# happyxtt/CNNs_SLFP_quantization

Measured on AMD Instinct MI355X. Metric: images/sec at batch 256, MobileNetV1 SLFP<3,4> ImageNet-224; % HBM roofline, higher is better.
Workload: dtype f32 (1x1 contraction: fp16 MFMA operands, f32 accumulate); 1 GPU; mobilenetv1_imagenet224: all 27 Conv2d_Q layers, SLFP<3,4> Qbits=8, NHWC, batch 256 per GPU as 2 concurrent image groups of 128 on 2 HIP streams, inputs resident in HBM; batch_per_gpu=256, global_batch=256, parallelism=batch-sharded x1, one-time RCCL broadcast of the u8 weight codes, pointwise_mfma=pw_mfma_f16x1

## Files before the change

cnns_slfp_quantization_amd/_lib.py:

```python
import ctypes
import os

_HERE = os.path.dirname(os.path.abspath(__file__))
LIB_PATH = os.path.join(_HERE, "libslfp_hip.so")

OK, ERR_BAD_ARG, ERR_SHAPE, ERR_UNSUPPORTED, ERR_ALIGNMENT, ERR_HIP = 0, -1, -2, -3, -4, -5
FMT_ACT8, FMT_W8, FMT_SFP7, FMT_EXT = 0, 1, 2, 4
LAYOUT_NCHW, LAYOUT_NHWC = 0, 1
BWD_DENSE = 1
MFMA_DEFAULT, MFMA_F16X1, MFMA_F16X3 = 0, 1, 3
OPT_SGD, OPT_DSGD, OPT_SSGD = 0, 1, 2

SYMBOLS = (
    "slfp_version", "slfp_last_error", "slfp_device_count",
    "slfp_encode_f32", "slfp_decode_f32", "slfp_quantize_f32", "slfp_quantize_layerout_f32", "slfp_absmax_f32",
    "slfp_conv2d_out_shape", "slfp_conv2d_kernel_name", "slfp_conv2d_wprep_bytes",
    "slfp_conv2d_prepare_weights", "slfp_conv2d_prepare_weights_codes", "slfp_conv2d_workspace_bytes", "slfp_conv2d_fwd", "slfp_conv2d_fwd_post",
    "slfp_linear_workspace_bytes", "slfp_linear_fwd", "slfp_linear_prepare_weights", "slfp_linear_fwd_prepared",
    "slfp_nchw_to_nhwc_f32", "slfp_nhwc_to_nchw_f32", "slfp_debug_div_mismatches",
    "slfp_debug_enc_mismatches", "slfp_enc_table_ok", "slfp_dwpw_supported", "slfp_dwpw_fwd",
    "slfp_conv2d_codes_supported", "slfp_conv2d_fwd_codes", "slfp_conv2d_fwd_codes_ws", "slfp_maxpool2d_codes", "slfp_debug_code_mismatches", "slfp_debug_reload_switches",
    "slfp_debug_enc_hl_mismatches", "slfp_sgd_step_f32", "slfp_debug_dw3x3_variant",
    "slfp_conv2d_bwd_supported", "slfp_conv2d_bwd_kernel_name", "slfp_conv2d_bwd_workspace_bytes", "slfp_conv2d_bwd",
    "slfp_conv2d_bwd_supported_ex", "slfp_conv2d_bwd_kernel_name_ex", "slfp_conv2d_bwd_workspace_bytes_ex", "slfp_conv2d_bwd_ex",
    "slfp_conv2d_res_supported", "slfp_conv2d_fwd_res",
    "slfp_conv2d_codes_slice_supported", "slfp_conv2d_fwd_codes_slice", "slfp_maxpool2d_codes_ex", "slfp_maxpool2d_out_shape",
    "slfp_conv2d_entry_supported", "slfp_conv2d_fwd_entry",
)


class ConvDesc(ctypes.Structure):
    _fields_ = [
        ("n", ctypes.c_int64), ("c_in", ctypes.c_int64), ("h", ctypes.c_int64), ("w", ctypes.c_int64),
        ("c_out", ctypes.c_int64), ("kh", ctypes.c_int64), ("kw", ctypes.c_int64),
        ("stride_h", ctypes.c_int32), ("stride_w", ctypes.c_int32), ("pad_h", ctypes.c_int32),
        ("pad_w", ctypes.c_int32), ("dil_h", ctypes.c_int32), ("dil_w", ctypes.c_int32),
        ("groups", ctypes.c_int32), ("x_layout", ctypes.c_int32), ("y_layout", ctypes.c_int32),
# ... 33 lines not shown
    L = ctypes.CDLL(LIB_PATH)
    vp, sz, ci, cf, i64 = ctypes.c_void_p, ctypes.c_size_t, ctypes.c_int, ctypes.c_float, ctypes.c_int64
    dp = ctypes.POINTER(ConvDesc)
    sigs = {
        "slfp_version": (ci, []),
        "slfp_last_error": (ctypes.c_char_p, []),
        "slfp_device_count": (ci, []),
        "slfp_encode_f32": (ci, [vp, vp, sz, cf, ci, vp]),
        "slfp_decode_f32": (ci, [vp, vp, sz, ci, vp]),
        "slfp_quantize_f32": (ci, [vp, vp, sz, cf, ci, vp]),
        "slfp_quantize_layerout_f32": (ci, [vp, vp, sz, vp]),
        "slfp_absmax_f32": (ci, [vp, sz, vp, vp]),
        "slfp_conv2d_out_shape": (ci, [dp, ctypes.POINTER(i64), ctypes.POINTER(i64)]),
        "slfp_conv2d_kernel_name": (ctypes.c_char_p, [dp]),
        "slfp_debug_dw3x3_variant": (ctypes.c_char_p, [dp, ci]),
        "slfp_conv2d_wprep_bytes": (sz, [dp]),
        "slfp_conv2d_prepare_weights": (ci, [dp, vp, vp, vp, vp]),
        "slfp_conv2d_prepare_weights_codes": (ci, [dp, vp, vp, vp, vp]),
        "slfp_conv2d_workspace_bytes": (sz, [dp]),
        "slfp_conv2d_fwd": (ci, [dp, vp, vp, vp, vp, vp, vp, vp]),
        "slfp_conv2d_fwd_post": (ci, [dp, vp, vp, vp, vp, vp, ci, vp, vp, vp, vp]),
        "slfp_linear_workspace_bytes": (sz, [i64, i64, i64]),
        "slfp_linear_fwd": (ci, [vp, vp, vp, vp, i64, i64, i64, cf, cf, ci, ci, vp, vp]),
        "slfp_linear_prepare_weights": (ci, [vp, vp, i64, i64, cf, ci, ci, vp]),
        "slfp_linear_fwd_prepared": (ci, [vp, vp, vp, vp, i64, i64, i64, cf, cf, ci, ci, vp]),
        "slfp_nchw_to_nhwc_f32": (ci, [vp, vp, i64, i64, i64, i64, vp]),
        "slfp_nhwc_to_nchw_f32": (ci, [vp, vp, i64, i64, i64, i64, vp]),
        "slfp_debug_div_mismatches": (ci, [cf, vp, vp]),
        "slfp_debug_enc_mismatches": (ci, [cf, ci, vp, vp]),
        "slfp_enc_table_ok": (ci, [cf, ci]),
# ... 48 lines not shown
```

cnns_slfp_quantization_amd/csrc/codec.hip:

```cpp
#include <cstdarg>
#include <mutex>
#include <map>
#include <set>
#include <utility>
#include <cstdio>
#include "slfp_device.hpp"
#include "slfp_enc.hpp"
#include "slfp_host.hpp"

namespace slfp {

static thread_local char g_err[512] = "";

void set_error(const char* fmt, ...) {
    va_list ap;
    va_start(ap, fmt);
    vsnprintf(g_err, sizeof(g_err), fmt, ap);
    va_end(ap);
}

int fail(int code, const char* fmt, ...) {
    va_list ap;
    va_start(ap, fmt);
    vsnprintf(g_err, sizeof(g_err), fmt, ap);
// ... 36 lines not shown
    e = std::getenv("SLFP_PW_NT_MIN_MB");
    w.pw_nt_min_mb = e ? atoll(e) : 0;
    e = std::getenv("SLFP_DW_NT_MIN_MB");
    w.dw_nt_min_mb = e ? atoll(e) : 30;
    w.stem_old = std::getenv("SLFP_STEM_OLD") != nullptr;
    w.pwc_slice = std::getenv("SLFP_PWC_NOSLICE") == nullptr;
    w.dense_generic = std::getenv("SLFP_DENSE_GENERIC") != nullptr;
    e = std::getenv("SLFP_DENSE_CFG");
    w.dense_cfg = e ? atoi(e) : 0;
    e = std::getenv("SLFP_DENSE_NWB");
    w.dense_nwb = e ? atoi(e) : 0;
    w.dense_res = std::getenv("SLFP_DENSE_NORES") == nullptr;
    w.dense_encx = std::getenv("SLFP_DENSE_NOENCX") == nullptr;
    w.stem_im2row = std::getenv("SLFP_STEM_IM2ROW") != nullptr;
    w.dw_rows = parse_dw_rows(std::getenv("SLFP_DW_ROWS"));
    e = std::getenv("SLFP_PW_STREAM_MAX_KB");
    w.pw_stream_max_kb = e ? atoi(e) : 30;
    return w;
}
static Switches g_switches = read_switches();
const Switches& switches() { return g_switches; }
void reload_switches() { g_switches = read_switches(); }

int device_cu_count() {
    static std::mutex mu;
    static std::map<int, int> cus;
    int dev = 0;
    if (hipGetDevice(&dev) != hipSuccess) { (void)hipGetLastError(); return 256; }
    std::lock_guard<std::mutex> lock(mu);
    const auto it = cus.find(dev);
// ... 305 lines not shown
```

cnns_slfp_quantization_amd/csrc/conv_abi.hip:

```cpp
#include <cstring>
#include "slfp_device.hpp"
#include "slfp_codes.hpp"
#include "slfp_host.hpp"

namespace slfp {

static size_t round256(size_t b) { return (b + 255) & ~(size_t)255; }

static int make_plan_core(const slfp_conv2d_desc* d, ConvPlan* plan) {
    if (!d || !plan) return fail(SLFP_ERR_BAD_ARG, "conv2d: null descriptor");
    if (d->n <= 0 || d->c_in <= 0 || d->h <= 0 || d->w <= 0 || d->c_out <= 0 || d->kh <= 0 || d->kw <= 0)
        return fail(SLFP_ERR_SHAPE, "conv2d: non-positive size");
    if (d->stride_h <= 0 || d->stride_w <= 0 || d->dil_h <= 0 || d->dil_w <= 0 || d->pad_h < 0 || d->pad_w < 0)
        return fail(SLFP_ERR_SHAPE, "conv2d: bad stride/dilation/padding");
    if (d->groups <= 0 || d->c_in % d->groups || d->c_out % d->groups)
        return fail(SLFP_ERR_SHAPE, "conv2d: groups=%d does not divide C_in=%lld / C_out=%lld", d->groups,
                    (long long)d->c_in, (long long)d->c_out);
    if (d->qbits != 8 && d->qbits != 7)
        return fail(SLFP_ERR_BAD_ARG, "conv2d: qbits must be 8 (SLFP<3,4>) or 7 (SFP<3,3>), got %d", d->qbits);
    if ((d->x_layout != SLFP_LAYOUT_NCHW && d->x_layout != SLFP_LAYOUT_NHWC) ||
        (d->y_layout != SLFP_LAYOUT_NCHW && d->y_layout != SLFP_LAYOUT_NHWC))
        return fail(SLFP_ERR_BAD_ARG, "conv2d: unknown layout");
    if (!(d->ka > 0.f) || !(d->kw_scale > 0.f)) return fail(SLFP_ERR_BAD_ARG, "conv2d: Ka and Kw must be > 0");
    if (!scale_div_ok(d->ka) || !scale_div_ok(d->kw_scale))
// ... 219 lines not shown
const char* slfp_conv2d_kernel_name(const slfp_conv2d_desc* d) {
    ConvPlan p;
    if (make_plan(d, &p) != SLFP_OK) return "invalid";
    return family_name(p, *d);
}

const char* slfp_debug_dw3x3_variant(const slfp_conv2d_desc* d, int has_post) {
    ConvPlan p;
    if (make_plan(d, &p) != SLFP_OK || p.family != kDw3x3) return "none";
    static const float one = 1.f;
    const PostOp post = {has_post ? &one : nullptr, has_post ? &one : nullptr, 0, 0};
    if (dw3x3_rows_applicable(*d, p, nullptr, post)) return "rows";
    return dw3x3_tile_applicable(*d, p, nullptr, post) ? "tile" : "general";
}

size_t slfp_conv2d_wprep_bytes(const slfp_conv2d_desc* d) {
    ConvPlan p;
    if (make_plan(d, &p) != SLFP_OK) return 0;
    return p.wprep_bytes;
}

int slfp_conv2d_prepare_weights(const slfp_conv2d_desc* d, const float* w_oihw, void* wprep, float* weight_q_oihw,
                                void* stream) {
    ConvPlan p;
    const int rc = make_plan(d, &p);
    if (rc != SLFP_OK) return rc;
    if (!w_oihw || !wprep) return fail(SLFP_ERR_BAD_ARG, "slfp_conv2d_prepare_weights: null pointer");
    if (!aligned16(wprep)) return fail(SLFP_ERR_ALIGNMENT, "slfp_conv2d_prepare_weights: wprep must be 16-byte aligned");
    return launch_prepare_weights(*d, p, w_oihw, wprep, weight_q_oihw, as_stream(stream));
}
// ... 394 lines not shown
```

cnns_slfp_quantization_amd/csrc/conv_pw.hip:

```cpp
#include <cstdlib>
#include "slfp_device.hpp"
#include "slfp_enc.hpp"
#include "slfp_codes.hpp"
#include "slfp_host.hpp"
#include "conv_pw_params.hpp"

namespace slfp {

__device__ __forceinline__ half8 enc_frag(const float4 a, const float4 b, const EncArgs& e, const unsigned char* tb) {
    const uint2 pa = enc4_f16_raw(a, e.r1, e.lo, e.hi, tb), pb = enc4_f16_raw(b, e.r1, e.lo, e.hi, tb);
    typedef uint32_t u32x4 __attribute__((ext_vector_type(4)));
    return __builtin_bit_cast(half8, u32x4{pa.x, pa.y, pb.x, pb.y});
}
__device__ __forceinline__ half8 enc_frag_nan(const float4 a, const float4 b, const EncArgs& e, const unsigned char* tb) {
    const uint2 pa = enc4_f16(a, e.r1, e.lo, e.hi, tb), pb = enc4_f16(b, e.r1, e.lo, e.hi, tb);
    typedef uint32_t u32x4 __attribute__((ext_vector_type(4)));
    return __builtin_bit_cast(half8, u32x4{pa.x, pa.y, pb.x, pb.y});
}

__device__ __forceinline__ void enc_frag_hl(const float4 a, const float4 b, const EncArgs& e, const unsigned char* tb,
                                            const unsigned char* tl, half8& h, half8& l) {
    typedef uint32_t u32x4 __attribute__((ext_vector_type(4)));
    uint32_t h0, h1, h2, h3, l0, l1, l2, l3;
    enc2_f16_hl(a.x, a.y, e.r1, e.lo, e.hi, tb, tl, h0, l0);
// ... 247 lines not shown
                float4 r = tile_out(j);
                if constexpr (RES) r = res_add(r, rc, p.post.relu);
                const int n = j * 16 + kq * 4;
                if constexpr (A8) {
                    if (live && n < p.N) *reinterpret_cast<float2*>(yr + j * 16) = make_float2(r.x, r.y);
                    if (live && n + 2 < p.N) *reinterpret_cast<float2*>(yr + j * 16 + 2) = make_float2(r.z, r.w);
                } else {
                    if (live && n < p.N) st_stream4<SLFP_NT_PW>(yr + j * 16, r);
                }
            }
        }
    }
}


template <int FMT, int PASSES, int WM, int WN, int MT, int NT, bool KFULL, bool TAB = false, bool STG = false, bool RES = false, bool YC = false>
__global__ __launch_bounds__(64 * WM * WN, (WM * WN) <= 4 ? 2 : 4) void k_pw_tiled(const PwParams p) {
    static_assert(!STG || NT == 4, "the staged epilogue stores a wave's 64 channels per row");
    static_assert(!RES || STG, "residual operand: staged epilogue only");
    static_assert(!YC || (TAB && !STG && !RES && PASSES == 1 && NT == 4), "code output: single-pass table kernels, four channel tiles per wave");
    constexpr int TABB = TAB ? kPwTab : 64;
    constexpr int TABL = (TAB && (PASSES == 3 || YC)) ? kPwTab : 16;
    constexpr int T = 64 * WM * WN;
    constexpr int BM = WM * MT * 16;
    constexpr int BN = WN * NT * 16;
    constexpr int NLD = BM * 16 / T;
    static_assert(BM * 16 % T == 0, "staging must divide evenly");
    constexpr int XBYTES = BM * 128;

    __shared__ __attribute__((aligned(16))) unsigned char stab[TABB];
    __shared__ __attribute__((aligned(16))) unsigned char stab_lo[TABL];
    extern __shared__ __attribute__((aligned(16))) unsigned char smem[];
    uint32_t* sT = reinterpret_cast<uint32_t*>(stab);
    unsigned char* xs = smem;
    if constexpr (TAB) enc_fill<T>(reinterpret_cast<uint2*>(stab), p.enc);
    else lut_fill<FMT>(sT);
    if constexpr (TAB && (PASSES == 3 || YC)) enc_fill_compact<T>(reinterpret_cast<uint2*>(stab_lo), p.enc_lo);

    const uint32_t b = xcd_remap(blockIdx.x, p.nblocks);
    const uint32_t nb = b % p.n_blocks, mb = b / p.n_blocks;
    const int64_t m0 = (int64_t)mb * p.rb;
    const int lane = threadIdx.x & 63, wave = threadIdx.x >> 6;
    const int wm = wave / WN, wn = wave % WN;
    const int col = lane & 15, kq = lane >> 4;

    const int kc = threadIdx.x & 15;
    const int st_chunk = (kc >> 3) * 4 + (kc & 3);
    const uint32_t st_sub = (uint32_t)((kc & 7) >> 2) * 8u;
    const float* src[NLD];
#pragma unroll
    for (int i = 0; i < NLD; ++i) {
        const int row = (threadIdx.x >> 4) + i * (T / 16);
        int64_t m = m0 + (row < p.rb ? row : p.rb - 1);
        m = m < p.M ? m : p.M - 1;
        src[i] = p.x + x_row_offset(p, m) + kc * 4;
    }

    float4 st[NLD];
    auto load_stage = [&](int t) {
#ifdef SLFP_ABL_NOX
        if (t >= 2) {
#pragma unroll
            for (int i = 0; i < NLD; ++i) asm volatile("" : "+v"(st[i].x), "+v"(st[i].y), "+v"(st[i].z), "+v"(st[i].w));
            return;
        }
#endif
#pragma unroll
        for (int i = 0; i < NLD; ++i) {
            if constexpr (KFULL) {
                st[i] = ld_stream4<SLFP_NT_PWT>(src[i] + t * 64);
            } else {
                const int k = t * 64 + kc * 4;
                const int kk = k < p.K ? t * 64 : p.K - 4 - kc * 4;
                st[i] = *reinterpret_cast<const float4*>(src[i] + kk);
                if (k >= p.K) st[i] = make_float4(0.f, 0.f, 0.f, 0.f);
            }
        }
    };
    auto encode_store = [&](int buf) {
        unsigned char* hi = xs + (size_t)buf * (PASSES == 3 ? 2 : 1) * XBYTES;
        unsigned char* lo = hi + XBYTES;
#pragma unroll
        for (int i = 0; i < NLD; ++i) {
            const int row = (threadIdx.x >> 4) + i * (T / 16);
            const uint32_t off = lds_x_off(row, st_chunk) + st_sub;
            if constexpr (TAB && PASSES == 3) {
                uint2 ph, pl;
                enc2_f16_hl(st[i].x, st[i].y, p.enc.r1, p.enc.lo, p.enc.hi, stab, stab_lo, ph.x, pl.x);
                enc2_f16_hl(st[i].z, st[i].w, p.enc.r1, p.enc.lo, p.enc.hi, stab, stab_lo, ph.y, pl.y);
                if (__builtin_expect(enc_has_nan4(st[i]), 0)) enc_patch_nan4_f16(st[i], ph);
                *reinterpret_cast<uint2*>(hi + off) = ph;
                *reinterpret_cast<uint2*>(lo + off) = pl;
            } else if constexpr (TAB) {
#ifdef SLFP_ABL_NOENC
// ... 23 lines not shown
    const int ntile0 = (int)nb * (BN / 16) + wn * NT;
    const size_t wplane = (size_t)(p.wlo - p.whi);
    const int wn_u = __builtin_amdgcn_readfirstlane(wn);
    const int ntile0u = (int)nb * (BN / 16) + wn_u * NT;
    const uint64_t wbytes = (uint64_t)p.n_tiles * p.KS * 1024;
    const uint32_t wrecs = (uint32_t)(wbytes > 0xFFFFFFFFull ? 0xFFFFFFFFull : wbytes);
    const __amdgpu_buffer_rsrc_t rwh = __builtin_amdgcn_make_buffer_rsrc(const_cast<_Float16*>(p.whi), 0, wrecs, 0x00020000);
    const __amdgpu_buffer_rsrc_t rwl = __builtin_amdgcn_make_buffer_rsrc(const_cast<_Float16*>(PASSES == 3 ? p.wlo : p.whi), 0, wrecs, 0x00020000);
    uint32_t wsoff[NT];
#pragma unroll
    for (int j = 0; j < NT; ++j) {
        const int nt = ntile0u + j < p.n_tiles ? ntile0u + j : p.n_tiles - 1;
        wsoff[j] = (uint32_t)nt * (uint32_t)p.KS * 1024u;
    }
    const uint32_t wvoff = (uint32_t)lane * 16u;
    half8 wh[NT], wl[NT];
    auto load_w = [&](int kstep) {
#ifdef SLFP_ABL_NOW
        if (kstep >= 1) {
#pragma unroll
            for (int j = 0; j < NT; ++j) asm volatile("" : "+v"(wh[j]));
            return;
        }
#endif
#pragma unroll
        for (int j = 0; j < NT; ++j) {
            typedef uint32_t u32x4w __attribute__((ext_vector_type(4)));
            const uint32_t so = wsoff[j] + (uint32_t)kstep * 1024u;
            wh[j] = __builtin_bit_cast(half8, __builtin_amdgcn_raw_buffer_load_b128(rwh, wvoff, so, 0));
            if constexpr (PASSES == 3) wl[j] = __builtin_bit_cast(half8, __builtin_amdgcn_raw_buffer_load_b128(rwl, wvoff, so, 0));
        }
    };
    auto mfma_step = [&](int buf, int ks) {
        const unsigned char* hi = xs + (size_t)buf * (PASSES == 3 ? 2 : 1) * XBYTES;
        const unsigned char* lo = hi + XBYTES;
#pragma unroll
        for (int i = 0; i < MT; ++i) {
            const int row = (wm * MT + i) * 16 + col;
            const uint32_t off = lds_x_off(row, ks * 4 + kq);
            const half8 xh = *reinterpret_cast<const half8*>(hi + off);
            half8 xl;
            if constexpr (PASSES == 3) xl = *reinterpret_cast<const half8*>(lo + off);
#pragma unroll
            for (int j = 0; j < NT; ++j) {
                if constexpr (PASSES == 3) {
                    acc[i][j] = __builtin_amdgcn_mfma_f32_16x16x32_f16(wl[j], xh, acc[i][j], 0, 0, 0);
                    acc[i][j] = __builtin_amdgcn_mfma_f32_16x16x32_f16(wh[j], xl, acc[i][j], 0, 0, 0);
                }
#ifdef SLFP_ABL_NOMFMA
                asm volatile("" :: "v"(wh[j]), "v"(xh));
#else
                acc[i][j] = __builtin_amdgcn_mfma_f32_16x16x32_f16(wh[j], xh, acc[i][j], 0, 0, 0);
#endif
            }
        }
    };

    SLFP_STAMP(0);
    __syncthreads();
    SLFP_STAMP(1);
    load_stage(0);
    encode_store(0);
    load_stage(KT > 1 ? 1 : 0);
    __syncthreads();
    SLFP_STAMP(2);

    for (int t = 0; t + 1 < KT; ++t) {
        const int buf = t & 1;
#ifdef SLFP_PW_STAMPS2
        if (t == 3) SLFP_STAMP(3);
#endif
        load_w(t * 2);
        encode_store(buf ^ 1);
        load_stage(t + 2 < KT ? t + 2 : KT - 1);
#ifdef SLFP_PW_STAMPS2
        if (t == 3) { asm volatile("s_waitcnt lgkmcnt(0)" ::: "memory"); SLFP_STAMP(4); }
#endif
        mfma_step(buf, 0);
#ifdef SLFP_PW_STAMPS2
        if (t == 3) { asm volatile("s_nop 0" : "+v"(acc[0][0]), "+v"(acc[3][3])); SLFP_STAMP(5); }
#endif
        load_w(t * 2 + 1);
        mfma_step(buf, 1);
#ifdef SLFP_PW_STAMPS2
        if (t == 3) { asm volatile("s_nop 0" : "+v"(acc[0][0]), "+v"(acc[3][3])); SLFP_STAMP(6); }
#endif
        __syncthreads();
#ifdef SLFP_PW_STAMPS2
        if (t == 3) SLFP_STAMP(7);
#else
        SLFP_STAMP(3 + (t < 8 ? t : 8));
#endif
    }
    SLFP_STAMP(12);
    const int srow = lane >> 4, sch = lane & 15;
    const int n_st = ntile0 * 16 + sch * 4;
    const uint64_t yleft = (uint64_t)(p.M - m0) * p.N * 4;
    const uint32_t ybytes = (uint32_t)(yleft > 0xFFFFFFFFull ? 0xFFFFFFFFull : yleft);
    auto piece = [&](int i, int h) {
        const int row = (wm * MT + i) * 16 + h * 4 + srow;
        const bool ok = row < p.rb && m0 + row < p.M && n_st < p.N;
        return ok ? (uint32_t)(row * p.N + n_st) * 4u : 0xFFFFFFF0u;
    };
    const __amdgpu_buffer_rsrc_t rr = __builtin_amdgcn_make_buffer_rsrc(const_cast<float*>(RES ? p.res : p.y) + (size_t)m0 * p.N, 0, ybytes, 0x00020000);
    u32x4r rq[4];
    {
        const int t = KT - 1, buf = t & 1;
        load_w(t * 2);
        mfma_step(buf, 0);
        load_w(t * 2 + 1);
        if constexpr (RES) {
#pragma unroll
            for (int h = 0; h < 4; ++h) rq[h] = res_load_stg(rr, piece(0, h));
        }
        mfma_step(buf, 1);
    }

    const int n_lo = (int)nb * BN;
    float* lsc = reinterpret_cast<float*>(xs);
    float* lsh = lsc + BN;
    if (p.post.scale) {
        __syncthreads();
        for (int i = threadIdx.x; i < BN; i += T) {
            const bool in = n_lo + i < p.N;
            lsc[i] = in ? p.post.scale[n_lo + i] : 1.f;
            lsh[i] = in ? p.post.shift[n_lo + i] : 0.f;
        }
        __syncthreads();
    }
    SLFP_STAMP(13);
    if constexpr (YC) {
        const float r1 = p.enc_lo.r1, lo = p.enc_lo.lo, hi = p.enc_lo.hi;
#pragma unroll
        for (int i = 0; i < MT; ++i) {
            uint32_t c[NT];
#pragma unroll
            for (int j = 0; j < NT; ++j) {
// ... 7 lines not shown
                    r.z = __builtin_fmaf(r.z, sc.z, sh.z); r.w = __builtin_fmaf(r.w, sc.w, sh.w);
                }
                if (p.sgn) c[j] = code_sign4(enc4_code<false>(r, r1, lo, hi, stab_lo), r, p.fmt_out);
                else c[j] = enc4_code_relu(relu_of_nan4(r), r1, lo, hi, stab_lo);
            }
            rows_transpose4(c[0], c[1], c[2], c[3]);
            const int row = (wm * MT + i) * 16 + col;
            const int n = (ntile0 + kq) * 16;
            typedef uint32_t u32x4 __attribute__((ext_vector_type(4)));
            if (row < p.rb && m0 + row < p.M && n < p.N)
                *reinterpret_cast<u32x4*>(p.yc + (size_t)(m0 + row) * p.N + n) = u32x4{c[0], c[1], c[2], c[3]};
        }
        return;
    }
    if constexpr (STG) {
        unsigned char* stg = xs + 2 * (PASSES == 3 ? 2 : 1) * XBYTES + wave * (16 * kStgRow);
        const __amdgpu_buffer_rsrc_t ry = __builtin_amdgcn_make_buffer_rsrc(p.y + (size_t)m0 * p.N, 0, ybytes, 0x00020000);
#pragma unroll
        for (int i = 0; i < MT; ++i) {
#pragma unroll
            for (int j = 0; j < NT; ++j) {
                const int n = (ntile0 + j) * 16 + kq * 4;
                const bool in = n < p.N;
                float4 r = epilogue(acc[i][j], in ? bias_q256(p, n) : make_float4(0.f, 0.f, 0.f, 0.f), p.s1x, p.s2);
                if (p.post.scale) {
                    const float4 sc = *reinterpret_cast<const float4*>(lsc + (in ? n - n_lo : 0));
                    const float4 sh = *reinterpret_cast<const float4*>(lsh + (in ? n - n_lo : 0));
                    r.x = __builtin_fmaf(r.x, sc.x, sh.x); r.y = __builtin_fmaf(r.y, sc.y, sh.y);
                    r.z = __builtin_fmaf(r.z, sc.z, sh.z); r.w = __builtin_fmaf(r.w, sc.w, sh.w);
                    if (p.post.layerout) r = layerout4(r);
                }
// ... 42 lines not shown
            if (p.post.scale) {
                const float4 sc = *reinterpret_cast<const float4*>(lsc + (n - n_lo));
                const float4 sh = *reinterpret_cast<const float4*>(lsh + (n - n_lo));
                r.x = __builtin_fmaf(r.x, sc.x, sh.x); r.y = __builtin_fmaf(r.y, sc.y, sh.y);
                r.z = __builtin_fmaf(r.z, sc.z, sh.z); r.w = __builtin_fmaf(r.w, sc.w, sh.w);
                if (p.post.layerout) r = layerout4(r);
            }
            if (p.post.relu) { r.x = fmaxf(r.x, 0.f); r.y = fmaxf(r.y, 0.f); r.z = fmaxf(r.z, 0.f); r.w = fmaxf(r.w, 0.f); }
            st_stream4<SLFP_NT_PW>(p.y + (size_t)m * p.N + n, r);
        }
    }
}


static int set_lds_limit(const void* fn, size_t lds) { return raise_lds_limit(fn, lds); }

template <int FMT, int PASSES, int WM, int WN, int MT, int NT, bool KFULL>
static int launch_tiled_k(PwParams& p, hipStream_t stream) {
    constexpr int BM = WM * MT * 16, BN = WN * NT * 16, T = 64 * WM * WN;
    p.n_blocks = (uint32_t)ceil_div((int64_t)p.N, BN);
    p.rb = BM;
    p.m_blocks = (uint32_t)ceil_div(p.M, p.rb);
    const int64_t nblocks = (int64_t)p.m_blocks * p.n_blocks;
    if (nblocks > 0x7FFFFFFF) return fail(SLFP_ERR_UNSUPPORTED, "pointwise: grid too large");
    p.nblocks = (uint32_t)nblocks;
    if (p.yc) {
        if constexpr (NT == 4 && PASSES == 1) {
            if (p.enc.valid && p.enc_lo.valid && !p.res) {
                const size_t lds = (size_t)2 * BM * 128;
                auto fn = k_pw_tiled<FMT, 1, WM, WN, MT, NT, KFULL, true, false, false, true>;
// ... 10 lines not shown
            if (p.enc.valid && (PASSES == 1 || p.enc_lo.valid) && !switches().pw_nostg) {
                const size_t lds = (size_t)2 * (PASSES == 3 ? 2 : 1) * BM * 128 + (size_t)(T / 64) * 16 * kStgRow;
                auto fn = k_pw_tiled<FMT, PASSES, WM, WN, MT, NT, KFULL, true, true, true>;
                int rc = set_lds_limit(reinterpret_cast<const void*>(fn), lds);
                if (rc != SLFP_OK) return rc;
                hipLaunchKernelGGL(fn, dim3(p.nblocks), dim3(T), lds, stream, p);
                return check_launch("slfp pointwise (tiled, residual) kernel");
            }
        }
        return fail(SLFP_ERR_UNSUPPORTED, "pointwise: no residual form of this kernel variant");
    }
    {
        if (p.enc.valid && (PASSES == 1 || p.enc_lo.valid)) {
            if constexpr (NT == 4) {
                if (!switches().pw_nostg) {
                    const size_t lds = (size_t)2 * (PASSES == 3 ? 2 : 1) * BM * 128 + (size_t)(T / 64) * 16 * kStgRow;
                    auto fn = k_pw_tiled<FMT, PASSES, WM, WN, MT, NT, KFULL, true, true>;
                    int rc = set_lds_limit(reinterpret_cast<const void*>(fn), lds);
                    if (rc != SLFP_OK) return rc;
                    hipLaunchKernelGGL(fn, dim3(p.nblocks), dim3(T), lds, stream, p);
                    return check_launch("slfp pointwise (tiled) kernel");
                }
            }
            const size_t lds = (size_t)2 * (PASSES == 3 ? 2 : 1) * BM * 128;
            auto fn = k_pw_tiled<FMT, PASSES, WM, WN, MT, NT, KFULL, true>;
            int rc = set_lds_limit(reinterpret_cast<const void*>(fn), lds);
            if (rc != SLFP_OK) return rc;
            hipLaunchKernelGGL(fn, dim3(p.nblocks), dim3(T), lds, stream, p);
            return check_launch("slfp pointwise (tiled) kernel");
        }
// ... 56 lines not shown
    int per_cu = resident_blocks_per_cu(reinterpret_cast<const void*>(fn), kStreamThreads, lds);
    per_cu = per_cu < 1 ? 1 : (per_cu > 4 ? 4 : per_cu);
    (void)lds_total;
    const int64_t groups = (p.M + 15) / 16;
    int64_t grid = (int64_t)device_cu_count() * per_cu;
    const int64_t need = ceil_div(groups, kStreamThreads / 64);
    if (grid > need) grid = need;
    hipLaunchKernelGGL(fn, dim3((unsigned)grid), dim3(kStreamThreads), lds, stream, p);
    return check_launch("slfp pointwise (stream) kernel");
}

bool pointwise_stream_fits(int64_t k_pad, int64_t n_pad, int passes) {
    const size_t w = (size_t)k_pad * n_pad * 2 * (passes == 3 ? 2 : 1);
    return k_pad <= 256 && w <= (size_t)128 * 1024;
}
static bool stream_fits(const ConvPlan& plan, int passes, const PwParams& p) {
    if (!pointwise_stream_fits(plan.k_pad, plan.n_pad, passes)) return false;
    if (p.K % 4 || p.N % 4) return true;
    const size_t w = (size_t)plan.k_pad * plan.n_pad * 2 * (passes == 3 ? 2 : 1);
    return w <= (size_t)(passes == 3 ? 100 : switches().pw_stream_max_kb) * 1024;
}

template <int FMT, int PASSES>
static int launch_pw(PwParams& p, const ConvPlan& plan, hipStream_t stream) {
    if (stream_fits(plan, PASSES, p)) {
        switch ((p.K + 31) / 32) {
            case 1: return launch_stream_ks<FMT, PASSES, 1>(p, stream);
            case 2: return launch_stream_ks<FMT, PASSES, 2>(p, stream);
            case 3: return launch_stream_ks<FMT, PASSES, 3>(p, stream);
            case 4: return launch_stream_ks<FMT, PASSES, 4>(p, stream);
            case 5: case 6: return launch_stream_ks<FMT, PASSES, 6>(p, stream);
            case 7: case 8: return launch_stream_ks<FMT, PASSES, 8>(p, stream);
            default: break;
        }
    }
    if (p.K % 4 || p.N % 4) return fail(SLFP_ERR_UNSUPPORTED, "pointwise: channel counts not a multiple of 4 need the stream kernel");
    if constexpr (PASSES == 3) {
        if (p.N > 128) return launch_tiled<FMT, 3, 1, 4, 4, 4>(p, stream);
        if (p.N > 64) return launch_tiled<FMT, 3, 2, 2, 2, 4>(p, stream);
        return launch_tiled<FMT, 3, 4, 1, 1, 4>(p, stream);
    } else {
        if (p.N > 256) return launch_tiled<FMT, 1, 1, 8, 4, 4>(p, stream);
        if (p.N > 128) return launch_tiled<FMT, 1, 1, 4, 4, 4>(p, stream);
        if (p.N > 64) return launch_tiled<FMT, 1, 2, 2, 2, 4>(p, stream);
        return launch_tiled<FMT, 1, 4, 1, 1, 4>(p, stream);
    }
}

bool pointwise_res_applicable(const slfp_conv2d_desc& d, const ConvPlan& plan) {
    if (plan.family != kPointwise || plan.repad || d.stride_h != 1 || d.stride_w != 1) return false;
    if (d.c_in % 4 || d.c_out % 4) return false;
    if (switches().pw_notab || switches().pw_nostg) return false;
    if (!act_table(d.ka, plan.fmt_act, kEncF16P)) return false;
    if (plan.passes == 3 && !act_table(d.ka, plan.fmt_act, kEncF16LO)) return false;
    return true;
}

bool pointwise_entry_applicable(const slfp_conv2d_desc& d, const ConvPlan& plan, int post_flags, float y_ka, int y_fmt) {
    if (plan.family != kPointwise || plan.repad || plan.passes != 1) return false;
    if (post_flags & SLFP_POST_LAYEROUT) return false;
    if (d.c_out % 16 || d.c_in % 4) return false;
    if (switches().pw_notab || !act_table(d.ka, plan.fmt_act, kEncF16P)) return false;
    const EncArgs* t = enc_table(y_ka, y_fmt, kEncCode);
    return t->valid && enc_compact_covers(*t);
}

static int launch_pointwise_any(const slfp_conv2d_desc& d, const ConvPlan& plan, const float* x, const void* wfrag, const float* bias,
                                const PostOp& post, float* y, hipStream_t stream, const float* res, uint8_t* yc, float y_ka, int y_fmt);

int launch_pointwise(const slfp_conv2d_desc& d, const ConvPlan& plan, const float* x, const void* wfrag,
// ... 55 lines not shown
```

cnns_slfp_quantization_amd/csrc/slfp_host.hpp:

```cpp
#pragma once
#include <hip/hip_runtime.h>
#include <stdint.h>
#include <stddef.h>
#include <cmath>
#include <cstring>
#include <cstdlib>
#include "../../include/slfp.h"
#include "slfp_device.hpp"
#include "slfp_enc.hpp"

namespace slfp {

void set_error(const char* fmt, ...);
int fail(int code, const char* fmt, ...);
int check_launch(const char* what);

int raise_lds_limit(const void* fn, size_t lds_bytes);

inline hipStream_t as_stream(void* s) { return reinterpret_cast<hipStream_t>(s); }
inline bool aligned16(const void* p) { return (reinterpret_cast<uintptr_t>(p) & 15u) == 0; }
inline int64_t ceil_div(int64_t a, int64_t b) { return (a + b - 1) / b; }

inline bool scale_div_ok(float d) { return std::isfinite(d) && d >= 1e-30f && d <= 1e30f; }

// ... 6 lines not shown

struct Switches {
    bool long_encode, dw_old, pw_nostg, pw_notab;
    int pw_stg_maxks;
    long long pw_nt_min_mb;
    long long dw_nt_min_mb;
    bool stem_old;
    bool pwc_slice;
    bool dense_generic;
    int dense_cfg;
    int dense_nwb;
    bool dense_encx;
    bool dense_res;
    bool stem_im2row;
    int dw_rows;
    int pw_stream_max_kb;
};
const Switches& switches();
void reload_switches();
inline bool long_encode_forced() { return switches().long_encode; }
inline bool dw_old_forced() { return switches().dw_old; }
inline const EncArgs* act_table(float ka, int fmt_act, int rep) {
    if (long_encode_forced()) return nullptr;
    const EncArgs* t = enc_table(ka, fmt_act, rep);
    return t->valid ? t : nullptr;
}

enum KernelFamily { kDw3x3 = 0, kPointwise = 1, kDirect = 2, kDenseMfma = 3, kStemMfma = 4, kStemSmall = 5 };

struct ConvPlan {
// ... 20 lines not shown
bool dw3x3_rows_applicable(const slfp_conv2d_desc& d, const ConvPlan& p, const float* bias, const PostOp& post);
int launch_dw3x3_rows(const slfp_conv2d_desc& d, const ConvPlan& p, const float* x, const float* wq9c,
                      const PostOp& post, float* y, hipStream_t stream);
inline int parse_dw_rows(const char* e) {
    if (!e || !*e) return -1;
    const long v = strtol(e, nullptr, 0);
    return v <= 0 ? 0 : (int)(v & 0xF);
}
inline int dw_rows_class(int64_t h_out, int64_t w_out) {
    const int64_t px = h_out * w_out;
    return px >= 56 * 56 ? 0 : (px >= 28 * 28 ? 1 : (px >= 14 * 14 ? 2 : 3));
}
int launch_pointwise(const slfp_conv2d_desc& d, const ConvPlan& p, const float* x, const void* wfrag,
                     const float* bias, const PostOp& post, float* y, hipStream_t stream, const float* res = nullptr);
bool pointwise_res_applicable(const slfp_conv2d_desc& d, const ConvPlan& p);
struct CodeIo {
    bool x_codes;
    bool y_codes;
    float y_ka;
    int y_fmt;
    int64_t y_ld = 0;
};
int resident_blocks_per_cu(const void* fn, int block_threads, size_t dynamic_lds);
int device_cu_count();
bool pointwise_entry_applicable(const slfp_conv2d_desc& d, const ConvPlan& p, int post_flags, float y_ka, int y_fmt);
int launch_pointwise_entry(const slfp_conv2d_desc& d, const ConvPlan& p, const float* x, const void* wfrag, const float* bias,
                           const PostOp& post, void* y_codes, const CodeIo& io, hipStream_t stream);
bool pwc_applicable(const slfp_conv2d_desc& d, const ConvPlan& p, int post_flags, bool y_codes);
int launch_pwc(const slfp_conv2d_desc& d, const ConvPlan& p, const uint8_t* x, const void* wfrag, const float* bias,
               const PostOp& post, void* y, bool y_codes, float y_ka, int y_fmt, hipStream_t stream, const float* res = nullptr,
// ... 44 lines not shown
```

include/slfp.h:

```cpp
#ifndef SLFP_H_
#define SLFP_H_

#include <stddef.h>
#include <stdint.h>

#ifdef __cplusplus
extern "C" {
#endif

#define SLFP_ABI_VERSION 1

#define SLFP_OK 0
#define SLFP_ERR_BAD_ARG (-1)
#define SLFP_ERR_SHAPE (-2)
#define SLFP_ERR_UNSUPPORTED (-3)
#define SLFP_ERR_ALIGNMENT (-4)
#define SLFP_ERR_HIP (-5)

#define SLFP_FMT_ACT8 0
#define SLFP_FMT_W8 1
#define SLFP_FMT_SFP7 2
#define SLFP_FMT_EXT 4

#define SLFP_LAYOUT_NCHW 0
// ... 19 lines not shown

typedef struct slfp_conv2d_desc {
    int64_t n, c_in, h, w;
    int64_t c_out, kh, kw;
    int32_t stride_h, stride_w, pad_h, pad_w, dil_h, dil_w, groups;
    int32_t x_layout, y_layout;
    int32_t qbits;
    float ka, kw_scale;
    int32_t mfma_passes;
    int32_t reserved;
} slfp_conv2d_desc;

int slfp_conv2d_out_shape(const slfp_conv2d_desc* d, int64_t* h_out, int64_t* w_out);
const char* slfp_conv2d_kernel_name(const slfp_conv2d_desc* d);
const char* slfp_debug_dw3x3_variant(const slfp_conv2d_desc* d, int has_post);

size_t slfp_conv2d_wprep_bytes(const slfp_conv2d_desc* d);
int slfp_conv2d_prepare_weights(const slfp_conv2d_desc* d, const float* w_oihw, void* wprep,
                                float* weight_q_oihw, void* stream);
int slfp_conv2d_prepare_weights_codes(const slfp_conv2d_desc* d, const uint8_t* codes_oihw, void* wprep,
                                      float* weight_q_oihw, void* stream);
size_t slfp_conv2d_workspace_bytes(const slfp_conv2d_desc* d);
int slfp_conv2d_fwd(const slfp_conv2d_desc* d, const float* x, const void* wprep, const float* bias,
                    float* y, float* input_q, void* workspace, void* stream);

#define SLFP_POST_RELU 1
#define SLFP_POST_LAYEROUT 2
int slfp_conv2d_fwd_post(const slfp_conv2d_desc* d, const float* x, const void* wprep, const float* bias,
                         const float* post_scale, const float* post_shift, int relu, float* y,
                         float* input_q, void* workspace, void* stream);
// ... 89 lines not shown
```

Before: 134,100 images/sec.

## Add short-K pointwise kernel variant and tighten launch bounds on tiled pointwise

Adds a short-K form of the tiled pointwise MFMA kernel for K of at most 256. It stages and encodes the whole K extent into LDS up front, then runs the MFMA steps with double-buffered weight registers and no per-step barriers. It also aliases the staging buffer for the epilogue. The variant is gated by SLFP_PW_SHORTK and a compile-time rule that defaults to off. Separately, the default tiled kernel now requests a higher minimum occupancy for the single-pass, four-wave, 16-fragment staged case, which caps its registers and risks spills. Its main loop also peels the final staged iteration to drop a redundant tail load. A debug query reports which pointwise variant a layer would use.

New measurement: 133,600 images/sec. Within noise of the previous version (-0.3%).

```diff
diff --git a/cnns_slfp_quantization_amd/_lib.py b/cnns_slfp_quantization_amd/_lib.py
--- a/cnns_slfp_quantization_amd/_lib.py
+++ b/cnns_slfp_quantization_amd/_lib.py
@@ -20,7 +20,7 @@
     "slfp_nchw_to_nhwc_f32", "slfp_nhwc_to_nchw_f32", "slfp_debug_div_mismatches",
     "slfp_debug_enc_mismatches", "slfp_enc_table_ok", "slfp_dwpw_supported", "slfp_dwpw_fwd",
     "slfp_conv2d_codes_supported", "slfp_conv2d_fwd_codes", "slfp_conv2d_fwd_codes_ws", "slfp_maxpool2d_codes", "slfp_debug_code_mismatches", "slfp_debug_reload_switches",
-    "slfp_debug_enc_hl_mismatches", "slfp_sgd_step_f32", "slfp_debug_dw3x3_variant",
+    "slfp_debug_enc_hl_mismatches", "slfp_sgd_step_f32", "slfp_debug_dw3x3_variant", "slfp_debug_pw_variant",
     "slfp_conv2d_bwd_supported", "slfp_conv2d_bwd_kernel_name", "slfp_conv2d_bwd_workspace_bytes", "slfp_conv2d_bwd",
     "slfp_conv2d_bwd_supported_ex", "slfp_conv2d_bwd_kernel_name_ex", "slfp_conv2d_bwd_workspace_bytes_ex", "slfp_conv2d_bwd_ex",
     "slfp_conv2d_res_supported", "slfp_conv2d_fwd_res",
@@ -84,6 +84,7 @@
         "slfp_conv2d_out_shape": (ci, [dp, ctypes.POINTER(i64), ctypes.POINTER(i64)]),
         "slfp_conv2d_kernel_name": (ctypes.c_char_p, [dp]),
         "slfp_debug_dw3x3_variant": (ctypes.c_char_p, [dp, ci]),
+        "slfp_debug_pw_variant": (ctypes.c_char_p, [dp]),
         "slfp_conv2d_wprep_bytes": (sz, [dp]),
         "slfp_conv2d_prepare_weights": (ci, [dp, vp, vp, vp, vp]),
         "slfp_conv2d_prepare_weights_codes": (ci, [dp, vp, vp, vp, vp]),
diff --git a/cnns_slfp_quantization_amd/csrc/codec.hip b/cnns_slfp_quantization_amd/csrc/codec.hip
--- a/cnns_slfp_quantization_amd/csrc/codec.hip
+++ b/cnns_slfp_quantization_amd/csrc/codec.hip
@@ -74,6 +74,7 @@
     w.dense_encx = std::getenv("SLFP_DENSE_NOENCX") == nullptr;
     w.stem_im2row = std::getenv("SLFP_STEM_IM2ROW") != nullptr;
     w.dw_rows = parse_dw_rows(std::getenv("SLFP_DW_ROWS"));
+    w.pw_shortk = parse_dw_rows(std::getenv("SLFP_PW_SHORTK"));
     e = std::getenv("SLFP_PW_STREAM_MAX_KB");
     w.pw_stream_max_kb = e ? atoi(e) : 30;
     return w;
diff --git a/cnns_slfp_quantization_amd/csrc/conv_abi.hip b/cnns_slfp_quantization_amd/csrc/conv_abi.hip
--- a/cnns_slfp_quantization_amd/csrc/conv_abi.hip
+++ b/cnns_slfp_quantization_amd/csrc/conv_abi.hip
@@ -257,6 +257,12 @@
     return dw3x3_tile_applicable(*d, p, nullptr, post) ? "tile" : "general";
 }
 
+const char* slfp_debug_pw_variant(const slfp_conv2d_desc* d) {
+    ConvPlan p;
+    if (make_plan(d, &p) != SLFP_OK) return "none";
+    return pointwise_variant(*d, p);
+}
+
 size_t slfp_conv2d_wprep_bytes(const slfp_conv2d_desc* d) {
     ConvPlan p;
     if (make_plan(d, &p) != SLFP_OK) return 0;
diff --git a/cnns_slfp_quantization_amd/csrc/conv_pw.hip b/cnns_slfp_quantization_amd/csrc/conv_pw.hip
--- a/cnns_slfp_quantization_amd/csrc/conv_pw.hip
+++ b/cnns_slfp_quantization_amd/csrc/conv_pw.hip
@@ -285,11 +285,16 @@
 }
 
 
-template <int FMT, int PASSES, int WM, int WN, int MT, int NT, bool KFULL, bool TAB = false, bool STG = false, bool RES = false, bool YC = false>
-__global__ __launch_bounds__(64 * WM * WN, (WM * WN) <= 4 ? 2 : 4) void k_pw_tiled(const PwParams p) {
+constexpr int pw_tiled_min_waves(int passes, int waves, int frags, bool stg_f32) {
+    return waves > 4 ? 4 : ((passes == 1 && waves == 4 && frags == 16 && stg_f32) ? 4 : 2);
+}
+
+template <int FMT, int PASSES, int WM, int WN, int MT, int NT, bool KFULL, bool TAB = false, bool STG = false, bool RES = false, bool YC = false, int SKT = 0>
+__global__ __launch_bounds__(64 * WM * WN, pw_tiled_min_waves(PASSES, WM * WN, MT * NT, STG && !RES && !YC)) void k_pw_tiled(const PwParams p) {
     static_assert(!STG || NT == 4, "the staged epilogue stores a wave's 64 channels per row");
     static_assert(!RES || STG, "residual operand: staged epilogue only");
     static_assert(!YC || (TAB && !STG && !RES && PASSES == 1 && NT == 4), "code output: single-pass table kernels, four channel tiles per wave");
+    static_assert(SKT == 0 || (SKT <= 4 && TAB && STG && KFULL && !RES && !YC && PASSES == 1), "short-K form: single-pass table kernels, staged epilogue, K = 64 SKT");
     constexpr int TABB = TAB ? kPwTab : 64;
     constexpr int TABL = (TAB && (PASSES == 3 || YC)) ? kPwTab : 16;
     constexpr int T = 64 * WM * WN;
@@ -298,13 +303,16 @@
     constexpr int NLD = BM * 16 / T;
     static_assert(BM * 16 % T == 0, "staging must divide evenly");
     constexpr int XBYTES = BM * 128;
+    constexpr int NXB = SKT > 0 ? SKT : 2 * (PASSES == 3 ? 2 : 1);
+    constexpr bool SK_ALIAS = SKT > 2;
 
     __shared__ __attribute__((aligned(16))) unsigned char stab[TABB];
     __shared__ __attribute__((aligned(16))) unsigned char stab_lo[TABL];
     extern __shared__ __attribute__((aligned(16))) unsigned char smem[];
     uint32_t* sT = reinterpret_cast<uint32_t*>(stab);
     unsigned char* xs = smem;
-    if constexpr (TAB) enc_fill<T>(reinterpret_cast<uint2*>(stab), p.enc);
+    if constexpr (SKT > 0) { }
+    else if constexpr (TAB) enc_fill<T>(reinterpret_cast<uint2*>(stab), p.enc);
     else lut_fill<FMT>(sT);
     if constexpr (TAB && (PASSES == 3 || YC)) enc_fill_compact<T>(reinterpret_cast<uint2*>(stab_lo), p.enc_lo);
 
@@ -327,8 +335,7 @@
         src[i] = p.x + x_row_offset(p, m) + kc * 4;
     }
 
-    float4 st[NLD];
-    auto load_stage = [&](int t) {
+    auto load_stage = [&](float4 (&st)[NLD], int t) {
 #ifdef SLFP_ABL_NOX
         if (t >= 2) {
 #pragma unroll
@@ -348,7 +355,7 @@
             }
         }
     };
-    auto encode_store = [&](int buf) {
+    auto encode_store = [&](const float4 (&st)[NLD], int buf) {
         unsigned char* hi = xs + (size_t)buf * (PASSES == 3 ? 2 : 1) * XBYTES;
         unsigned char* lo = hi + XBYTES;
 #pragma unroll
@@ -402,8 +409,7 @@
         wsoff[j] = (uint32_t)nt * (uint32_t)p.KS * 1024u;
     }
     const uint32_t wvoff = (uint32_t)lane * 16u;
-    half8 wh[NT], wl[NT];
-    auto load_w = [&](int kstep) {
+    auto load_w = [&](half8 (&wh)[NT], half8 (&wl)[NT], int kstep) {
 #ifdef SLFP_ABL_NOW
         if (kstep >= 1) {
 #pragma unroll
@@ -419,7 +425,7 @@
             if constexpr (PASSES == 3) wl[j] = __builtin_bit_cast(half8, __builtin_amdgcn_raw_buffer_load_b128(rwl, wvoff, so, 0));
         }
     };
-    auto mfma_step = [&](int buf, int ks) {
+    auto mfma_step = [&](const half8 (&wh)[NT], const half8 (&wl)[NT], int buf, int ks) {
         const unsigned char* hi = xs + (size_t)buf * (PASSES == 3 ? 2 : 1) * XBYTES;
         const unsigned char* lo = hi + XBYTES;
 #pragma unroll
@@ -444,41 +450,97 @@
         }
     };
 
-    SLFP_STAMP(0);
-    __syncthreads();
-    SLFP_STAMP(1);
-    load_stage(0);
-    encode_store(0);
-    load_stage(KT > 1 ? 1 : 0);
-    __syncthreads();
-    SLFP_STAMP(2);
-
-    for (int t = 0; t + 1 < KT; ++t) {
-        const int buf = t & 1;
+    if constexpr (SKT > 0) {
+        constexpr int SB = (8 / NLD) < SKT ? (8 / NLD) : SKT;
+        float4 sx[SB][NLD];
+        half8 wa[NT], wb[NT];
+        constexpr int NTE = (kEncEntries + T - 1) / T;
+        uint2 te[NTE];
+#pragma unroll
+        for (int j = 0; j < NTE; ++j) {
+            const int e = (int)threadIdx.x + j * T;
+            te[j] = p.enc.e[e < kEncEntries ? e : kEncEntries - 1];
+        }
+#pragma unroll
+        for (int s = 0; s < SB; ++s) load_stage(sx[s], s);
+        load_w(wa, wa, 0);
+#pragma unroll
+        for (int j = 0; j < NTE; ++j) {
+            const int e = (int)threadIdx.x + j * T;
+            reinterpret_cast<uint2*>(stab)[e < kEncEntries ? e : kEncEntries - 1] = te[j];
+        }
+        __syncthreads();
+#pragma unroll
+        for (int s0 = 0; s0 < SKT; s0 += SB) {
+#pragma unroll
+            for (int s = 0; s < SB; ++s)
+                if (s0 + s < SKT) encode_store(sx[s], s0 + s);
+#pragma unroll
+            for (int s = 0; s < SB; ++s)
+                if (s0 + SB + s < SKT) load_stage(sx[s], s0 + SB + s);
+        }
+        __syncthreads();
+#pragma unroll
+        for (int ks = 0; ks < 2 * SKT; ++ks) {
+            if (ks & 1) {
+                if (ks + 1 < 2 * SKT) load_w(wa, wa, ks + 1);
+                __builtin_amdgcn_sched_barrier(0);
+                mfma_step(wb, wb, ks >> 1, 1);
+            } else {
+                load_w(wb, wb, ks + 1);
+                __builtin_amdgcn_sched_barrier(0);
+                mfma_step(wa, wa, ks >> 1, 0);
+            }
+        }
+    }
+    float4 st[NLD];
+    half8 wh[NT], wl[NT];
+    if constexpr (SKT == 0) {
+        SLFP_STAMP(0);
+        __syncthreads();
+        SLFP_STAMP(1);
+        load_stage(st, 0);
+        encode_store(st, 0);
+        if (KT > 1) load_stage(st, 1);
+        __syncthreads();
+        SLFP_STAMP(2);
+
+        for (int t = 0; t + 2 < KT; ++t) {
+            const int buf = t & 1;
 #ifdef SLFP_PW_STAMPS2
-        if (t == 3) SLFP_STAMP(3);
-#endif
-        load_w(t * 2);
-        encode_store(buf ^ 1);
-        load_stage(t + 2 < KT ? t + 2 : KT - 1);
+            if (t == 3) SLFP_STAMP(3);
+#endif
+            load_w(wh, wl, t * 2);
+            encode_store(st, buf ^ 1);
+            load_stage(st, t + 2);
 #ifdef SLFP_PW_STAMPS2
-        if (t == 3) { asm volatile("s_waitcnt lgkmcnt(0)" ::: "memory"); SLFP_STAMP(4); }
-#endif
-        mfma_step(buf, 0);
+            if (t == 3) { asm volatile("s_waitcnt lgkmcnt(0)" ::: "memory"); SLFP_STAMP(4); }
+#endif
+            mfma_step(wh, wl, buf, 0);
 #ifdef SLFP_PW_STAMPS2
-        if (t == 3) { asm volatile("s_nop 0" : "+v"(acc[0][0]), "+v"(acc[3][3])); SLFP_STAMP(5); }
-#endif
-        load_w(t * 2 + 1);
-        mfma_step(buf, 1);
+            if (t == 3) { asm volatile("s_nop 0" : "+v"(acc[0][0]), "+v"(acc[3][3])); SLFP_STAMP(5); }
+#endif
+            load_w(wh, wl, t * 2 + 1);
+            mfma_step(wh, wl, buf, 1);
 #ifdef SLFP_PW_STAMPS2
-        if (t == 3) { asm volatile("s_nop 0" : "+v"(acc[0][0]), "+v"(acc[3][3])); SLFP_STAMP(6); }
-#endif
-        __syncthreads();
+            if (t == 3) { asm volatile("s_nop 0" : "+v"(acc[0][0]), "+v"(acc[3][3])); SLFP_STAMP(6); }
+#endif
+            __syncthreads();
 #ifdef SLFP_PW_STAMPS2
-        if (t == 3) SLFP_STAMP(7);
+            if (t == 3) SLFP_STAMP(7);
 #else
-        SLFP_STAMP(3 + (t < 8 ? t : 8));
-#endif
+            SLFP_STAMP(3 + (t < 8 ? t : 8));
+#endif
+        }
+        if (KT > 1) {
+            const int t = KT - 2, buf = t & 1;
+            load_w(wh, wl, t * 2);
+            encode_store(st, buf ^ 1);
+            mfma_step(wh, wl, buf, 0);
+            load_w(wh, wl, t * 2 + 1);
+            mfma_step(wh, wl, buf, 1);
+            __syncthreads();
+        }
     }
     SLFP_STAMP(12);
     const int srow = lane >> 4, sch = lane & 15;
@@ -492,23 +554,23 @@
     };
     const __amdgpu_buffer_rsrc_t rr = __builtin_amdgcn_make_buffer_rsrc(const_cast<float*>(RES ? p.res : p.y) + (size_t)m0 * p.N, 0, ybytes, 0x00020000);
     u32x4r rq[4];
-    {
+    if constexpr (SKT == 0) {
         const int t = KT - 1, buf = t & 1;
-        load_w(t * 2);
-        mfma_step(buf, 0);
-        load_w(t * 2 + 1);
+        load_w(wh, wl, t * 2);
+        mfma_step(wh, wl, buf, 0);
+        load_w(wh, wl, t * 2 + 1);
         if constexpr (RES) {
 #pragma unroll
             for (int h = 0; h < 4; ++h) rq[h] = res_load_stg(rr, piece(0, h));
         }
-        mfma_step(buf, 1);
+        mfma_step(wh, wl, buf, 1);
     }
 
     const int n_lo = (int)nb * BN;
     float* lsc = reinterpret_cast<float*>(xs);
     float* lsh = lsc + BN;
+    if (SK_ALIAS || p.post.scale) __syncthreads();
     if (p.post.scale) {
-        __syncthreads();
         for (int i = threadIdx.x; i < BN; i += T) {
             const bool in = n_lo + i < p.N;
             lsc[i] = in ? p.post.scale[n_lo + i] : 1.f;
@@ -546,7 +608,7 @@
         return;
     }
     if constexpr (STG) {
-        unsigned char* stg = xs + 2 * (PASSES == 3 ? 2 : 1) * XBYTES + wave * (16 * kStgRow);
+        unsigned char* stg = xs + (SK_ALIAS ? 2 * BN * 4 : NXB * XBYTES) + wave * (16 * kStgRow);
         const __amdgpu_buffer_rsrc_t ry = __builtin_amdgcn_make_buffer_rsrc(p.y + (size_t)m0 * p.N, 0, ybytes, 0x00020000);
 #pragma unroll
         for (int i = 0; i < MT; ++i) {
@@ -619,6 +681,25 @@
 
 
 static int set_lds_limit(const void* fn, size_t lds) { return raise_lds_limit(fn, lds); }
+
+constexpr int kPwShortKRule = 0;
+static bool shortk_class_on(int64_t K) {
+    if (K % 64 || K > 256) return false;
+    const int sw = switches().pw_shortk;
+    return (((sw < 0) ? kPwShortKRule : sw) >> (K / 64 - 1)) & 1;
+}
+
+template <int FMT, int WM, int WN, int MT, int NT, int SKT>
+static int launch_tiled_sk(PwParams& p, hipStream_t stream) {
+    constexpr int BM = WM * MT * 16, BN = WN * NT * 16, T = 64 * WM * WN;
+    constexpr size_t xb = (size_t)SKT * BM * 128, stgb = (size_t)(T / 64) * 16 * kStgRow;
+    constexpr size_t lds = SKT > 2 ? (xb > 2 * BN * 4 + stgb ? xb : 2 * BN * 4 + stgb) : xb + stgb;
+    auto fn = k_pw_tiled<FMT, 1, WM, WN, MT, NT, true, true, true, false, false, SKT>;
+    int rc = set_lds_limit(reinterpret_cast<const void*>(fn), lds);
+    if (rc != SLFP_OK) return rc;
+    hipLaunchKernelGGL(fn, dim3(p.nblocks), dim3(T), lds, stream, p);
+    return check_launch("slfp pointwise (tiled, short K) kernel");
+}
 
 template <int FMT, int PASSES, int WM, int WN, int MT, int NT, bool KFULL>
 static int launch_tiled_k(PwParams& p, hipStream_t stream) {
@@ -659,6 +740,16 @@
         if (p.enc.valid && (PASSES == 1 || p.enc_lo.valid)) {
             if constexpr (NT == 4) {
                 if (!switches().pw_nostg) {
+                    if constexpr (PASSES == 1 && KFULL && BM == 64 && BN >= 128) {
+                        if (shortk_class_on(p.K)) {
+                            switch (p.K / 64) {
+                                case 1: return launch_tiled_sk<FMT, WM, WN, MT, NT, 1>(p, stream);
+                                case 2: return launch_tiled_sk<FMT, WM, WN, MT, NT, 2>(p, stream);
+                                case 3: return launch_tiled_sk<FMT, WM, WN, MT, NT, 3>(p, stream);
+                                default: return launch_tiled_sk<FMT, WM, WN, MT, NT, 4>(p, stream);
+                            }
+                        }
+                    }
                     const size_t lds = (size_t)2 * (PASSES == 3 ? 2 : 1) * BM * 128 + (size_t)(T / 64) * 16 * kStgRow;
                     auto fn = k_pw_tiled<FMT, PASSES, WM, WN, MT, NT, KFULL, true, true>;
                     int rc = set_lds_limit(reinterpret_cast<const void*>(fn), lds);
@@ -745,16 +836,16 @@
     const size_t w = (size_t)k_pad * n_pad * 2 * (passes == 3 ? 2 : 1);
     return k_pad <= 256 && w <= (size_t)128 * 1024;
 }
-static bool stream_fits(const ConvPlan& plan, int passes, const PwParams& p) {
+static bool stream_fits(const ConvPlan& plan, int passes, int64_t K, int64_t N) {
     if (!pointwise_stream_fits(plan.k_pad, plan.n_pad, passes)) return false;
-    if (p.K % 4 || p.N % 4) return true;
+    if (K % 4 || N % 4) return true;
     const size_t w = (size_t)plan.k_pad * plan.n_pad * 2 * (passes == 3 ? 2 : 1);
     return w <= (size_t)(passes == 3 ? 100 : switches().pw_stream_max_kb) * 1024;
 }
 
 template <int FMT, int PASSES>
 static int launch_pw(PwParams& p, const ConvPlan& plan, hipStream_t stream) {
-    if (stream_fits(plan, PASSES, p)) {
+    if (stream_fits(plan, PASSES, p.K, p.N)) {
         switch ((p.K + 31) / 32) {
             case 1: return launch_stream_ks<FMT, PASSES, 1>(p, stream);
             case 2: return launch_stream_ks<FMT, PASSES, 2>(p, stream);
@@ -785,6 +876,15 @@
     if (!act_table(d.ka, plan.fmt_act, kEncF16P)) return false;
     if (plan.passes == 3 && !act_table(d.ka, plan.fmt_act, kEncF16LO)) return false;
     return true;
+}
+
+const char* pointwise_variant(const slfp_conv2d_desc& d, const ConvPlan& plan) {
+    if (plan.family != kPointwise || plan.repad) return "none";
+    const int passes = (plan.fmt_act == kFmtSfp7 || plan.passes != 3) ? 1 : 3;
+    if (stream_fits(plan, passes, d.c_in, d.c_out)) return "stream";
+    if (passes != 1 || d.c_out <= 64 || switches().pw_notab || switches().pw_nostg) return "tiled";
+    if (!act_table(d.ka, plan.fmt_act, kEncF16P)) return "tiled";
+    return shortk_class_on(d.c_in) ? "tiled_shortk" : "tiled";
 }
 
 bool pointwise_entry_applicable(const slfp_conv2d_desc& d, const ConvPlan& plan, int post_flags, float y_ka, int y_fmt) {
diff --git a/cnns_slfp_quantization_amd/csrc/slfp_host.hpp b/cnns_slfp_quantization_amd/csrc/slfp_host.hpp
--- a/cnns_slfp_quantization_amd/csrc/slfp_host.hpp
+++ b/cnns_slfp_quantization_amd/csrc/slfp_host.hpp
@@ -44,6 +44,7 @@
     bool dense_res;
     bool stem_im2row;
     int dw_rows;
+    int pw_shortk;
     int pw_stream_max_kb;
 };
 const Switches& switches();
@@ -94,6 +95,7 @@
 int launch_pointwise(const slfp_conv2d_desc& d, const ConvPlan& p, const float* x, const void* wfrag,
                      const float* bias, const PostOp& post, float* y, hipStream_t stream, const float* res = nullptr);
 bool pointwise_res_applicable(const slfp_conv2d_desc& d, const ConvPlan& p);
+const char* pointwise_variant(const slfp_conv2d_desc& d, const ConvPlan& p);
 struct CodeIo {
     bool x_codes;
     bool y_codes;
diff --git a/include/slfp.h b/include/slfp.h
--- a/include/slfp.h
+++ b/include/slfp.h
@@ -57,6 +57,7 @@
 int slfp_conv2d_out_shape(const slfp_conv2d_desc* d, int64_t* h_out, int64_t* w_out);
 const char* slfp_conv2d_kernel_name(const slfp_conv2d_desc* d);
 const char* slfp_debug_dw3x3_variant(const slfp_conv2d_desc* d, int has_post);
+const char* slfp_debug_pw_variant(const slfp_conv2d_desc* d);
 
 size_t slfp_conv2d_wprep_bytes(const slfp_conv2d_desc* d);
 int slfp_conv2d_prepare_weights(const slfp_conv2d_desc* d, const float* w_oihw, void* wprep,
```
